# zju3dv/LoFTR

Hardware: AMD Instinct MI355X
Metric: image-pairs/sec @640x480 indoor-ds (higher is better)
Workload: dtype f32; 1 GPU; batch=8 640x480 synthetic grayscale pairs per GPU, indoor_ds dual-softmax (BASELINE configs[1]), full LoFTR.forward = ResNet-FPN backbone (HIP implicit-GEMM / patch convolutions incl. the 7x7 stem) + HIP matching path; weights=seeded random init (no checkpoint on the box), conf_matrix_materialised=True, match_type=dual_softmax, global_batch=8, parallelism=dp1 (pairs sharded; RCCL all-gather of match counts)

## Files before the change

loftr_amd/csrc/common.h:

```cpp
#pragma once
#include <hip/hip_runtime.h>
#include <stdint.h>
#include <stddef.h>
#include "../../include/loftr_hip.h"

typedef float f32x16 __attribute__((ext_vector_type(16)));
typedef float f32x4 __attribute__((ext_vector_type(4)));
typedef float f32x2 __attribute__((ext_vector_type(2)));

#define LOFTR_NEG_INF (-1e9f)

#define LOFTR_CHECK_ARG(cond) do { if (!(cond)) return LOFTR_ERR_BAD_ARG; } while (0)
#define LOFTR_CHECK_LAUNCH() do { if (hipGetLastError() != hipSuccess) return LOFTR_ERR_LAUNCH; } while (0)

#ifdef __HIP_DEVICE_COMPILE__
#define LOFTR_NO_PACKED_FP32 __attribute__((target("no-packed-fp32-ops")))
#else
#define LOFTR_NO_PACKED_FP32
#endif

__host__ __device__ static inline int ceil_div(int a, int b) { return (a + b - 1) / b; }
static inline size_t align_up(size_t x, size_t a) { return (x + a - 1) / a * a; }

enum LoftrTimedKernel {
  LOFTR_T_SCORE_STATS = 0,
  LOFTR_T_SCORE_CONF = 1,
  LOFTR_T_PROJ = 2,
  LOFTR_T_LINEAR = 3,
  LOFTR_T_LINEAR_LN = 4,
  LOFTR_T_KV = 5,
  LOFTR_T_ATTN_APPLY = 6,
  LOFTR_T_ATTN_SMALL = 7,
  LOFTR_T_GATHER = 8,
  LOFTR_T_OT_STORE = 9,
  LOFTR_T_CONV = 10,
  LOFTR_T_CONV3 = 11,
  LOFTR_T_CONV3W = 12,
  LOFTR_T_ENCODER_X = 13,
  LOFTR_T_FINE_PAIR = 14,
  LOFTR_T_COUNT = 15
};
enum LoftrDebugKey {
  LOFTR_DBG_ENCODER_SCHEDULE = 0,
  LOFTR_DBG_CONV_PERSIST_CAP,
  LOFTR_DBG_WGRAD_CHUNK,
  LOFTR_DBG_REDUCE_TALL,
  LOFTR_DBG_PCT_GRID,
  LOFTR_DBG_PCT_SKIP,
  LOFTR_DBG_PCT_QUOTA,
  LOFTR_DBG_CONV_DUO,
  LOFTR_DBG_CONV_PATCH,
  LOFTR_DBG_CONV_REM,
  LOFTR_DBG_FINE_WAVES,
  LOFTR_DBG_COUNT
};
int loftr_debug_value(int key);
extern unsigned g_loftr_timing_mask;
extern int g_loftr_range_check;
void loftr_timing_mark(int id, hipStream_t st, bool end);
struct TimedLaunch {
  int id; hipStream_t st; bool on;
  TimedLaunch(int id_, hipStream_t st_) : id(id_), st(st_), on((g_loftr_timing_mask >> id_) & 1u) {
    if (on) loftr_timing_mark(id, st, false);
  }
  ~TimedLaunch() { if (on) loftr_timing_mark(id, st, true); }
};

constexpr int NUM_XCD = 8;
static inline unsigned xcd_grid(int tiles_m, int tiles_n) { return (unsigned)(NUM_XCD * ceil_div(tiles_m, NUM_XCD) * tiles_n); }
__device__ __forceinline__ bool xcd_tile(int tiles_m, int tiles_n, int& tile_m, int& tile_n) {
  const int id = blockIdx.x, xcd = id % NUM_XCD, slot = id / NUM_XCD;
  const int chunk = ceil_div(tiles_m, NUM_XCD);
  tile_n = slot % tiles_n;
  const int local = slot / tiles_n;
  tile_m = xcd * chunk + local;
  return local < chunk && tile_m < tiles_m;
}

struct WsAlloc {
  char* base; size_t cap; size_t off;
  WsAlloc(void* p, size_t bytes) : base((char*)p), cap(bytes), off(0) {}
  template <typename T> T* take(size_t n) {
    off = align_up(off, 256);
    T* r = (T*)(base + off);
    off += n * sizeof(T);
    return r;
  }
  bool ok() const { return off <= cap; }
};

__device__ __forceinline__ float wave_sum(float v) {
#pragma unroll
  for (int o = 32; o >= 1; o >>= 1) v += __shfl_xor(v, o, 64);
  return v;
}
__device__ __forceinline__ float wave_max(float v) {
#pragma unroll
  for (int o = 32; o >= 1; o >>= 1) v = fmaxf(v, __shfl_xor(v, o, 64));
  return v;
}
#define LOFTR_DPP(v_, ctrl_) __int_as_float(__builtin_amdgcn_update_dpp(0, __float_as_int(v_), ctrl_, 0xF, 0xF, true))
#define LOFTR_DPPI(v_, ctrl_) __builtin_amdgcn_update_dpp(0, v_, ctrl_, 0xF, 0xF, true)
__device__ __forceinline__ float half_sum(float v) {
  v += LOFTR_DPP(v, 0xB1);
  v += LOFTR_DPP(v, 0x4E);
  v += LOFTR_DPP(v, 0x141);
  v += LOFTR_DPP(v, 0x140);
  const auto r = __builtin_amdgcn_permlane16_swap(__float_as_int(v), __float_as_int(v), false, false);
  return __int_as_float(r[0]) + __int_as_float(r[1]);
}
__device__ __forceinline__ float half_max(float v) {
  v = fmaxf(v, LOFTR_DPP(v, 0xB1));
  v = fmaxf(v, LOFTR_DPP(v, 0x4E));
  v = fmaxf(v, LOFTR_DPP(v, 0x141));
  v = fmaxf(v, LOFTR_DPP(v, 0x140));
  const auto r = __builtin_amdgcn_permlane16_swap(__float_as_int(v), __float_as_int(v), false, false);
  return fmaxf(__int_as_float(r[0]), __int_as_float(r[1]));
}
__device__ __forceinline__ int half_min_i32(int v) {
  v = min(v, LOFTR_DPPI(v, 0xB1));
  v = min(v, LOFTR_DPPI(v, 0x4E));
  v = min(v, LOFTR_DPPI(v, 0x141));
  v = min(v, LOFTR_DPPI(v, 0x140));
  const auto r = __builtin_amdgcn_permlane16_swap(v, v, false, false);
  return min((int)r[0], (int)r[1]);
}
__device__ __forceinline__ void half_sum16(f32x16& v) {
#pragma unroll
  for (int r = 0; r < 16; ++r) v[r] += LOFTR_DPP(v[r], 0xB1);
#pragma unroll
  for (int r = 0; r < 16; ++r) v[r] += LOFTR_DPP(v[r], 0x4E);
#pragma unroll
  for (int r = 0; r < 16; ++r) v[r] += LOFTR_DPP(v[r], 0x141);
#pragma unroll
  for (int r = 0; r < 16; ++r) v[r] += LOFTR_DPP(v[r], 0x140);
#pragma unroll
  for (int r = 0; r < 16; ++r) {
    const auto q = __builtin_amdgcn_permlane16_swap(__float_as_int(v[r]), __float_as_int(v[r]), false, false);
    v[r] = __int_as_float(q[0]) + __int_as_float(q[1]);
// ... 27 lines not shown
```

loftr_amd/csrc/conv.hip:

```cpp
#include "gemm.h"
#include "conv_prepared.h"
#include <stdlib.h>

namespace {

using CfgD = GemmCfg<256, 128, 4, 2, 3>;

struct ConvArgs {
  ASrc a;
  const sp_t* w; int K;
  const float* bias;
  const float* wscale;
  const float* x_inv;
  const sp_t* residual;
  sp_t* y_sp;
  float* y_f32;
  int M, Cout, Coutp;
  int act;
  const sp_t* up;
  int Hl, Wl;
  float sy, sx;
};

template <typename Cfg, bool FULL>
__device__ __forceinline__ void conv_epilogue(const ConvArgs& p, f32x16 (&acc)[Cfg::TM][Cfg::TN], int m0, int n0) {
  const EpiLane<Cfg> e;
  const sp_t* rs = p.residual ? p.residual + (long)m0 * p.Coutp + n0 : nullptr;
  sp_t* os = p.y_sp ? p.y_sp + (long)m0 * p.Coutp + n0 : nullptr;
  float* of = p.y_f32 ? p.y_f32 + (long)m0 * p.Cout + n0 : nullptr;
#pragma unroll
  for (int j = 0; j < Cfg::TN; ++j) {
    const int col = n0 + e.lcol + j * 32;
    const bool creal = col < p.Cout;
    const bool cpad = col < p.Coutp;
    const float b = (p.bias && creal) ? p.bias[col] : 0.f;
    const float wsc = (creal ? p.wscale[col] : 1.f) * (p.x_inv ? *p.x_inv : 1.f);
#pragma unroll
    for (int i = 0; i < Cfg::TM; ++i) {
      f32x16 v = acc[i][j] * wsc;
      if (rs) {
        uint32_t w[16];
#pragma unroll
        for (int r = 0; r < 16; ++r) {
          const int trow = e.lrow + e.rr(i, r);
          const bool ok = (FULL || m0 + trow < p.M) && cpad;
          w[r] = ok ? rs[(unsigned)(trow * p.Coutp + e.spcol + j * 32)] : 0u;
        }
#pragma unroll
        for (int r = 0; r < 16; ++r) v[r] += sp_value(w[r], e.odd);
      }
#pragma unroll
      for (int r = 0; r < 16; ++r) {
        float x = v[r] + b;
        if (p.act == 1) x = fmaxf(x, 0.f);
        if (p.act == 2) x = x > 0.f ? x : 0.01f * x;
        v[r] = creal ? x : 0.f;
      }
      if (of) {
#pragma unroll
        for (int r = 0; r < 16; ++r) {
          const int trow = e.lrow + e.rr(i, r);
          if ((FULL || m0 + trow < p.M) && creal) of[(unsigned)(trow * p.Cout + e.lcol + j * 32)] = v[r];
        }
      }
      if (os) {
        uint32_t w[16];
        sp_words16(v, e.odd, w);
#pragma unroll
        for (int r = 0; r < 16; ++r) {
          const int trow = e.lrow + e.rr(i, r);
          if ((FULL || m0 + trow < p.M) && cpad) os[(unsigned)(trow * p.Coutp + e.spcol + j * 32)] = w[r];
        }
      }
    }
  }
}

template <typename Cfg>
__device__ __forceinline__ void conv_epilogue_up(const ConvArgs& p, f32x16 (&acc)[Cfg::TM][Cfg::TN], int m0, int n0,
                                                 float* lds) {
  constexpr int LD = Cfg::BN + 4;
  static_assert(Cfg::BM * LD <= Cfg::LDS_FLOATS, "accumulator tile does not fit the operand ring");
  const EpiLane<Cfg> e;
  __syncthreads();
  const float xinv = p.x_inv ? *p.x_inv : 1.f;
#pragma unroll
  for (int j = 0; j < Cfg::TN; ++j) {
    const int col = n0 + e.lcol + j * 32;
    const float wsc = (col < p.Cout ? p.wscale[col] : 1.f) * xinv;
#pragma unroll
    for (int i = 0; i < Cfg::TM; ++i)
#pragma unroll
      for (int r = 0; r < 16; ++r) lds[(e.lrow + e.rr(i, r)) * LD + e.lcol + j * 32] = acc[i][j][r] * wsc;
  }
  __syncthreads();
  const int Wo = 2 * p.Wl, Ho = 2 * p.Hl;
  constexpr int OCTS = Cfg::BN / 8;
  for (int it = threadIdx.x; it < Cfg::BM * OCTS; it += Cfg::THREADS) {
    const int row = it / OCTS, oct = it - row * OCTS;
    const int pix = m0 + row, col0 = n0 + oct * 8;
    if (pix >= p.M || col0 >= p.Coutp) continue;
    const int t = pix / Wo, x = pix - t * Wo;
    const int bb = t / Ho, y = t - bb * Ho;
    const float fy = p.sy * (float)y, fx = p.sx * (float)x;
    const int y0 = (int)fy, x0 = (int)fx;
    const int dy = y0 < p.Hl - 1 ? p.Wl * p.Coutp : 0, dx = x0 < p.Wl - 1 ? p.Coutp : 0;
    const float ly = fy - (float)y0, lx = fx - (float)x0;
    const float hy = 1.f - ly, hx = 1.f - lx;
    const int off = sp_octet_off(col0 >> 3);
    const sp_t* s00 = p.up + (unsigned)(((bb * p.Hl + y0) * p.Wl + x0) * p.Coutp + off);
    const sp_t* src[4] = {s00, s00 + dx, s00 + dy, s00 + dy + dx};
    u32x4 hi[4], lo[4];
#pragma unroll
    for (int k = 0; k < 4; ++k) {
      hi[k] = *reinterpret_cast<const u32x4*>(src[k]);
      lo[k] = *reinterpret_cast<const u32x4*>(src[k] + 16);
    }
    float v[4][8], o[8];
#pragma unroll
    for (int k = 0; k < 4; ++k) sp_unpack8(hi[k], lo[k], v[k]);
    const f32x4 a0 = *reinterpret_cast<const f32x4*>(&lds[row * LD + oct * 8]);
    const f32x4 a1 = *reinterpret_cast<const f32x4*>(&lds[row * LD + oct * 8 + 4]);
#pragma unroll
    for (int c = 0; c < 8; ++c)
      o[c] = col0 + c < p.Cout
                 ? (c < 4 ? a0[c] : a1[c - 4]) + (hy * (hx * v[0][c] + lx * v[1][c]) + ly * (hx * v[2][c] + lx * v[3][c]))
                 : 0.f;
    u32x4 oh, ol;
    sp_pack8(o, oh, ol);
    sp_t* dst = p.y_sp + (unsigned)(pix * p.Coutp + off);
    *reinterpret_cast<u32x4*>(dst) = oh;
    *reinterpret_cast<u32x4*>(dst + 16) = ol;
  }
}

template <typename Cfg, bool UP>
__global__ __launch_bounds__(Cfg::THREADS, 2) void conv_kernel(ConvArgs p) {
  __shared__ __attribute__((aligned(16))) float lds[Cfg::LDS_FLOATS];
  int tm, tn;
  if (!xcd_tile(ceil_div(p.M, Cfg::BM), ceil_div(p.Coutp, Cfg::BN), tm, tn)) return;
  const int m0 = tm * Cfg::BM, n0 = tn * Cfg::BN;
  f32x16 acc[Cfg::TM][Cfg::TN];
  gemm_mainloop<Cfg, true>(p.a, p.w, p.K, p.M, p.Cout, p.K, m0, n0, lds, acc, p.Coutp);
  if constexpr (UP) conv_epilogue_up<Cfg>(p, acc, m0, n0, lds);
  else if (m0 + Cfg::BM <= p.M) conv_epilogue<Cfg, true>(p, acc, m0, n0);
  else conv_epilogue<Cfg, false>(p, acc, m0, n0);
}

namespace c3 {
constexpr int TY = 8, TX = 32, PW = TX + 2, PH = TY + 2, PROWS = PW * PH;
constexpr int PSLOTS = 43, PQ = 6;
constexpr int PATCH_BYTES = PSLOTS * 1024, BTILE_BYTES = 128 * 128;
constexpr int NB = 4;
constexpr int LDS_BYTES = 2 * PATCH_BYTES + NB * BTILE_BYTES + 1024;
using Cfg = GemmCfg<256, 128, 4, 2, 3>;
}

struct Conv3Args {
  const sp_t* x; int B, H, W, Cp, Cin;
  const sp_t* w; int K;
  const float* bias; const float* wscale; const float* x_inv; const sp_t* residual; sp_t* y_sp; float* y_f32;
  int Cout, Coutp, act;
  const sp_t* zeros;
  int tiles_x, tiles_y;
  float* pbuf;
};

__global__ __launch_bounds__(512, 2) void conv3x3_kernel(Conv3Args p) {
  using namespace c3;
  typedef __attribute__((address_space(3))) void* lds_ptr_t;
  typedef const __attribute__((address_space(1))) void* gbl_ptr_t;
  __shared__ __attribute__((aligned(16))) char lds[LDS_BYTES];
  char* const patch_base = lds;
  char* const bring_base = lds + 2 * PATCH_BYTES;
  char* const scratch = lds + 2 * PATCH_BYTES + NB * BTILE_BYTES;

  const int tid = threadIdx.x, lane = tid & 63, wave = tid >> 6;
  const int wm = wave & 3, wn = wave >> 2;
  const int rsub = lane >> 3, slot = lane & 7;

  const int tiles_m = p.B * p.tiles_y * p.tiles_x, tiles_n = ceil_div(p.Coutp, 128);
  const int chunk_m = ceil_div(tiles_m, NUM_XCD), nvirt = NUM_XCD * chunk_m * tiles_n;
  int vid = blockIdx.x;
  int nb = 0, ny0 = 0, nx0 = 0, nn0 = 0;
  bool have = false;
#define C3_NEXT_TILE()                                                                                      \
  {                                                                                                         \
    have = false;                                                                                           \
    for (; vid < nvirt; vid += gridDim.x) {                                                                 \
      const int xcd__ = vid % NUM_XCD, slot__ = vid / NUM_XCD;                                              \
      const int local__ = slot__ / tiles_n, tm__ = xcd__ * chunk_m + local__;                               \
      if (local__ < chunk_m && tm__ < tiles_m) {                                                            \
        nb = tm__ / (p.tiles_y * p.tiles_x);                                                                \
        const int trem__ = tm__ - nb * (p.tiles_y * p.tiles_x);                                             \
        ny0 = (trem__ / p.tiles_x) * TY; nx0 = (trem__ % p.tiles_x) * TX; nn0 = (slot__ % tiles_n) * 128;   \
        have = true;                                                                                        \
        break;                                                                                              \
      }                                                                                                     \
    }                                                                                                       \
  }
  C3_NEXT_TILE()
  if (!have) return;

  int poff[PQ];
  int boff[2];
#define C3_DMA_OFFSETS()                                                                                    \
  {                                                                                                         \
    _Pragma("unroll") for (int q = 0; q < PQ; ++q) {                                                        \
      const int s = q * 8 + wave, r = s * 8 + rsub;                                                         \
      const int py = r / PW, px = r - py * PW;                                                              \
      const int gy = ny0 - 1 + py, gx = nx0 - 1 + px;                                                       \
      const bool in = s < PSLOTS && r < PROWS && (unsigned)gy < (unsigned)p.H && (unsigned)gx < (unsigned)p.W; \
      poff[q] = in ? ((nb * p.H + gy) * p.W + gx) * p.Cp + ((slot ^ ((r >> 1) & 7)) << 2) : -1;             \
    }                                                                                                       \
    _Pragma("unroll") for (int q = 0; q < 2; ++q) {                                                         \
      const int r = (q * 8 + wave) * 8 + rsub;                                                              \
      boff[q] = min(nn0 + r, p.Cout - 1) * p.K + ((slot ^ ((r >> 1) & 7)) << 2);                            \
    }                                                                                                       \
  }
  C3_DMA_OFFSETS()
  const int gpt = p.Cp >> 5, nk = 9 * gpt;

#define C3_ISSUE_PATCH(cg_, stage_)                                                                         \
  {                                                                                                         \
    _Pragma("unroll") for (int q = 0; q < PQ; ++q) {                                                        \
      const sp_t* g__ = poff[q] >= 0 ? p.x + (poff[q] + (cg_) * 32) : p.zeros;                              \
      char* d__ = (q * 8 + wave < PSLOTS) ? patch_base + (stage_) * PATCH_BYTES + (q * 8 + wave) * 1024 : scratch; \
      __builtin_amdgcn_global_load_lds((gbl_ptr_t)g__, (lds_ptr_t)d__, 16, 0, 0);                           \
    }                                                                                                       \
// ... 384 lines not shown
    cus = per_dev[dev];
  }
  return cus > 0 && nvirt > (unsigned)cus ? (unsigned)cus : nvirt;
}

template <int RT>
__global__ __launch_bounds__(256) void conv_rem_gather_kernel(const float* __restrict__ pbuf, long npix, int H, int W, int R, int c0, int Coutp,
                                                              const float* __restrict__ bias, const sp_t* __restrict__ residual, int act,
                                                              sp_t* __restrict__ y_sp) {
  const long pix = (long)blockIdx.x * 256 + threadIdx.x;
  if (pix >= npix) return;
  const int x = (int)(pix % W), y = (int)((pix / W) % H);
  float v[8];
#pragma unroll
  for (int c = 0; c < 8; ++c) v[c] = 0.f;
  const float* pp = pbuf + pix * (9 * R);
#pragma unroll
  for (int ky = 0; ky < 3; ++ky)
#pragma unroll
    for (int kx = 0; kx < 3; ++kx) {
      const int yy = y + ky - 1, xx = x + kx - 1;
      if ((unsigned)yy < (unsigned)H && (unsigned)xx < (unsigned)W) {
        const float* q = pp + ((long)(ky - 1) * W + (kx - 1)) * (9 * R) + (ky * 3 + kx) * R;
        if (RT == 4) {
          const f32x4 t = *reinterpret_cast<const f32x4*>(q);
          v[0] += t[0]; v[1] += t[1]; v[2] += t[2]; v[3] += t[3];
        } else {
#pragma unroll
          for (int c = 0; c < 7; ++c) if (c < R) v[c] += q[c];
        }
      }
    }
  sp_t* row = y_sp + pix * Coutp + c0;
  float rv[8];
#pragma unroll
  for (int c = 0; c < 8; ++c) rv[c] = 0.f;
  if (residual) {
    const sp_t* rr = residual + pix * Coutp + c0;
    const u32x4 hi = *reinterpret_cast<const u32x4*>(rr), lo = *reinterpret_cast<const u32x4*>(rr + 16);
    sp_unpack8(hi, lo, rv);
  }
  const float slope = act == 1 ? 0.f : act == 2 ? 0.01f : 1.f;
  float o[8];
#pragma unroll
  for (int c = 0; c < 8; ++c) {
    const float t = v[c] + ((bias && c < R) ? bias[c0 + c] : 0.f) + rv[c];
    o[c] = c < R ? fmaxf(t, slope * t) : 0.f;
  }
  u32x4 oh, ol;
  sp_pack8(o, oh, ol);
  const u32x4 z = {0u, 0u, 0u, 0u};
  u32x4* dst = reinterpret_cast<u32x4*>(row);
  dst[0] = oh; dst[1] = z; dst[2] = z; dst[3] = z; dst[4] = ol; dst[5] = z; dst[6] = z; dst[7] = z;
}


static int conv_prepare(const float* weight, const long* weight_strides, int Cin, int Cout, int KH, int KW,
                        const float* bn_weight, const float* bn_bias, const float* bn_mean, const float* bn_var, float bn_eps,
                        void* buf, size_t bytes, hipStream_t st) {
  LOFTR_CHECK_ARG(weight && weight_strides && buf && Cin > 0 && Cout > 0 && KH > 0 && KW > 0);
  LOFTR_CHECK_ARG((bn_weight == nullptr) == (bn_bias == nullptr) && (bn_weight == nullptr) == (bn_mean == nullptr) &&
                  (bn_weight == nullptr) == (bn_var == nullptr));
  ConvPrepared pr;
  if (!conv_prepared_layout(buf, bytes, Cin, Cout, KH, KW, pr)) return LOFTR_ERR_WORKSPACE;
  const int Cp = ceil32(Cin), K = KH * KW * Cp;
  (void)hipMemsetAsync(pr.zeros, 0, 256, st);
  hipLaunchKernelGGL(conv_rowscale_kernel, dim3(Cout), dim3(256), 0, st, weight, bn_weight, bn_bias, bn_mean, bn_var, bn_eps,
                     Cin, KH, KW, weight_strides[0], weight_strides[1], weight_strides[2], weight_strides[3], pr.bias, pr.wscale);
  hipLaunchKernelGGL(conv_prep_kernel, dim3(ceil_div(K / 32, 8), Cout), dim3(256), 0, st, weight, bn_weight, bn_bias,
                     bn_mean, bn_var, bn_eps, Cin, Cp, KH, KW, weight_strides[0], weight_strides[1], weight_strides[2],
                     weight_strides[3], pr.wsp, pr.wscale);
  LOFTR_CHECK_LAUNCH();
  return LOFTR_OK;
}

static int conv_rem_channels(int Cout, int KH, int KW, int stride) {
  return (KH == 3 && KW == 3 && stride == 1 && ceil32(Cout) == 224 && Cout - 192 >= 1 && Cout - 192 <= 7) ? Cout - 192 : 0;
}
extern "C" size_t loftr_conv_scratch_bytes(int B, int H, int W, int Cout, int KH, int KW, int stride) {
  const int R = conv_rem_channels(Cout, KH, KW, stride);
  return (R > 0 && B > 0 && H > 0 && W > 0) ? (size_t)B * H * W * 9 * R * 4 : 0;
}

static int conv_run(const uint32_t* x_sp, int B, int H, int W, int Cin, const void* prepared, size_t prepared_bytes, int Cout,
                    int KH, int KW, int stride, int pad, int act, const uint32_t* residual_sp, const uint32_t* up_sp,
                    uint32_t* y_sp, float* y_f32, void* stream, const float* x_inv = nullptr, void* scratch = nullptr, size_t scratch_bytes = 0) {
  LOFTR_CHECK_ARG(x_sp && prepared && (y_sp || y_f32) && B >= 0 && H > 0 && W > 0 && Cin > 0 && Cout > 0);
  const bool shared_gpu = (act & LOFTR_CONV_SHARED_GPU) != 0;
  act &= ~LOFTR_CONV_SHARED_GPU;
  LOFTR_CHECK_ARG(KH > 0 && KW > 0 && stride > 0 && pad >= 0 && act >= 0 && act <= 2);
  if (B == 0) return LOFTR_OK;
  hipStream_t st = (hipStream_t)stream;
  ConvGeom g;
  g.H = H; g.W = W; g.Cp = ceil32(Cin); g.KH = KH; g.KW = KW; g.stride = stride; g.pad = pad;
  g.Ho = (H + 2 * pad - KH) / stride + 1;
  g.Wo = (W + 2 * pad - KW) / stride + 1;
  if (g.Ho <= 0 || g.Wo <= 0 || H >= 32768 || W >= 32768) return LOFTR_ERR_UNSUPPORTED;
  if (up_sp && ((g.Ho & 1) || (g.Wo & 1) || KH != 1 || KW != 1 || stride != 1 || pad != 0 || !y_sp || y_f32 || residual_sp || act != 0))
    return LOFTR_ERR_UNSUPPORTED;
  const long M = (long)B * g.Ho * g.Wo;
  if (M * (long)ceil32(Cout) >= (1L << 31) || (long)B * H * W * g.Cp >= (1L << 31)) return LOFTR_ERR_UNSUPPORTED;
  const int K = KH * KW * g.Cp;
  ConvPrepared pr;
  if (!conv_prepared_layout(const_cast<void*>(prepared), prepared_bytes, Cin, Cout, KH, KW, pr)) return LOFTR_ERR_WORKSPACE;
  sp_t* wsp = pr.wsp;
  float* bias = pr.bias;
  sp_t* zeros = pr.zeros;
  g.zeros = zeros;
  ConvArgs p;
  p.a = asrc_conv(x_sp, g);
  p.w = wsp; p.K = K; p.bias = bias; p.wscale = pr.wscale; p.x_inv = x_inv; p.residual = residual_sp; p.y_sp = y_sp; p.y_f32 = y_f32;
  p.M = (int)M; p.Cout = Cout; p.Coutp = ceil32(Cout); p.act = act;
  p.up = up_sp; p.Hl = g.Ho / 2; p.Wl = g.Wo / 2;
  p.sy = g.Ho > 1 ? (float)(p.Hl - 1) / (float)(g.Ho - 1) : 0.f;
  p.sx = g.Wo > 1 ? (float)(p.Wl - 1) / (float)(g.Wo - 1) : 0.f;
  if (loftr_debug_value(LOFTR_DBG_CONV_PATCH) && KH == 3 && KW == 3 && stride == 1 && pad == 1 && !up_sp) {
    Conv3Args c;
    c.x = x_sp; c.B = B; c.H = H; c.W = W; c.Cp = g.Cp; c.Cin = Cin; c.w = wsp; c.K = K; c.bias = bias; c.wscale = pr.wscale; c.x_inv = x_inv; c.residual = residual_sp;
    c.y_sp = y_sp; c.y_f32 = y_f32; c.Cout = Cout; c.Coutp = ceil32(Cout); c.act = act; c.zeros = zeros;
    c.tiles_x = ceil_div(W, c3::TX); c.tiles_y = ceil_div(H, c3::TY); c.pbuf = nullptr;
    const bool duo = loftr_debug_value(LOFTR_DBG_CONV_DUO) != 0;
    const bool wide = duo && c.Coutp == 32 * 7;
    TimedLaunch tl(wide ? LOFTR_T_CONV3W : LOFTR_T_CONV3, st);
    if (duo && c.Coutp % 128 == 0) {
      using CF = c3d::Cfg<4, 2, 4>;
      c.tiles_y = ceil_div(H, CF::TY);
      hipLaunchKernelGGL((conv3x3_duo_kernel<CF>), dim3(xcd_grid(B * c.tiles_x * c.tiles_y, c.Coutp / 128)), dim3(256), 0, st, c);
    } else if (duo && c.Coutp == 192) {
      using CF = c3d::Cfg<6, 2, 4, 8, 2>;
      c.tiles_y = ceil_div(H, CF::TY);
      hipLaunchKernelGGL((conv3x3_duo_kernel<CF>), dim3(xcd_grid(B * c.tiles_x * c.tiles_y, 1)), dim3(512), 0, st, c);
    } else if (wide && conv_rem_channels(Cout, KH, KW, stride) > 0 && !y_f32 && loftr_debug_value(LOFTR_DBG_CONV_REM) &&
               scratch && scratch_bytes >= (size_t)B * H * W * 9 * conv_rem_channels(Cout, KH, KW, stride) * 4) {
      using CF = c3d::Cfg<6, 2, 4, 8, 2, true>;
      c.tiles_y = ceil_div(H, CF::TY);
      c.pbuf = reinterpret_cast<float*>(scratch);
      hipLaunchKernelGGL((conv3x3_duo_kernel<CF>), dim3(xcd_grid(B * c.tiles_x * c.tiles_y, 1)), dim3(512), 0, st, c);
      LOFTR_CHECK_LAUNCH();
      const long npix = (long)B * H * W;
      if (Cout - 192 == 4)
        hipLaunchKernelGGL(conv_rem_gather_kernel<4>, dim3((unsigned)((npix + 255) / 256)), dim3(256), 0, st, c.pbuf, npix, H, W, 4, 192, c.Coutp,
                           bias, residual_sp, act, y_sp);
      else
        hipLaunchKernelGGL(conv_rem_gather_kernel<0>, dim3((unsigned)((npix + 255) / 256)), dim3(256), 0, st, c.pbuf, npix, H, W, Cout - 192, 192, c.Coutp,
                           bias, residual_sp, act, y_sp);
    } else if (wide) {
      using CF = c3d::Cfg<7, 2, 4, 8, 2>;
      c.tiles_y = ceil_div(H, CF::TY);
      hipLaunchKernelGGL((conv3x3_duo_kernel<CF>), dim3(xcd_grid(B * c.tiles_x * c.tiles_y, 1)), dim3(512), 0, st, c);
    } else
      hipLaunchKernelGGL(conv3x3_kernel, dim3(shared_gpu ? xcd_grid(B * c.tiles_x * c.tiles_y, ceil_div(c.Coutp, 128))
                                                         : persistent_grid(xcd_grid(B * c.tiles_x * c.tiles_y, ceil_div(c.Coutp, 128)))),
                         dim3(512), 0, st, c);
    LOFTR_CHECK_LAUNCH();
    return LOFTR_OK;
  }
  {
    TimedLaunch tl(LOFTR_T_CONV, st);
    if (up_sp)
      hipLaunchKernelGGL((conv_kernel<CfgD, true>), dim3(xcd_grid(ceil_div(p.M, CfgD::BM), ceil_div(p.Coutp, CfgD::BN))),
                         dim3(CfgD::THREADS), 0, st, p);
    else
      hipLaunchKernelGGL((conv_kernel<CfgD, false>), dim3(xcd_grid(ceil_div(p.M, CfgD::BM), ceil_div(p.Coutp, CfgD::BN))),
                         dim3(CfgD::THREADS), 0, st, p);
  }
  LOFTR_CHECK_LAUNCH();
  return LOFTR_OK;
}

#ifdef LOFTR_CONV_PROBE
extern "C" int loftr_conv_probe_buffer(void* buf) {
  long long* b = (long long*)buf;
  return hipMemcpyToSymbol(HIP_SYMBOL(g_conv_probe), &b, sizeof(b)) == hipSuccess ? LOFTR_OK : LOFTR_ERR_LAUNCH;
}
#endif

extern "C" int loftr_conv_prepare(const float* weight, const long* weight_strides, int Cin, int Cout, int KH, int KW,
                                  const float* bn_weight, const float* bn_bias, const float* bn_mean, const float* bn_var,
                                  float bn_eps, void* prepared, size_t prepared_bytes, void* stream) {
  return conv_prepare(weight, weight_strides, Cin, Cout, KH, KW, bn_weight, bn_bias, bn_mean, bn_var, bn_eps, prepared,
                      prepared_bytes, (hipStream_t)stream);
}

extern "C" int loftr_conv_bn_act_prepared(const uint32_t* x_sp, int B, int H, int W, int Cin, const void* prepared,
                                          size_t prepared_bytes, int Cout, int KH, int KW, int stride, int pad, int act,
                                          const uint32_t* residual_sp, const uint32_t* low_sp, uint32_t* y_sp, float* y_f32,
                                          const float* x_inv_scale, void* stream) {
  return conv_run(x_sp, B, H, W, Cin, prepared, prepared_bytes, Cout, KH, KW, stride, pad, act, residual_sp, low_sp, y_sp, y_f32,
                  stream, x_inv_scale);
}

extern "C" int loftr_conv_bn_act_prepared_scratch(const uint32_t* x_sp, int B, int H, int W, int Cin, const void* prepared,
                                                  size_t prepared_bytes, int Cout, int KH, int KW, int stride, int pad, int act,
                                                  const uint32_t* residual_sp, const uint32_t* low_sp, uint32_t* y_sp, float* y_f32,
                                                  const float* x_inv_scale, void* scratch, size_t scratch_bytes, void* stream) {
  return conv_run(x_sp, B, H, W, Cin, prepared, prepared_bytes, Cout, KH, KW, stride, pad, act, residual_sp, low_sp, y_sp, y_f32,
                  stream, x_inv_scale, scratch, scratch_bytes);
}

extern "C" int loftr_conv_bn_act(const uint32_t* x_sp, int B, int H, int W, int Cin, const float* weight,
                                 const long* weight_strides, int Cout, int KH, int KW, int stride, int pad, const float* bn_weight, const float* bn_bias,
                                 const float* bn_mean, const float* bn_var, float bn_eps, int act,
                                 const uint32_t* residual_sp, uint32_t* y_sp, float* y_f32, void* ws, size_t ws_bytes,
                                 const float* x_inv_scale, void* stream) {
  LOFTR_CHECK_ARG(x_sp && (y_sp || y_f32) && B >= 0 && H > 0 && W > 0);
  if (B == 0) return LOFTR_OK;
  const int rc = conv_prepare(weight, weight_strides, Cin, Cout, KH, KW, bn_weight, bn_bias, bn_mean, bn_var, bn_eps, ws, ws_bytes,
                              (hipStream_t)stream);
  if (rc != LOFTR_OK) return rc;
  return conv_run(x_sp, B, H, W, Cin, ws, ws_bytes, Cout, KH, KW, stride, pad, act, residual_sp, nullptr, y_sp, y_f32, stream, x_inv_scale);
}

extern "C" int loftr_conv1x1_upsample_add(const uint32_t* x_sp, int B, int H, int W, int Cin, const float* weight,
                                          const long* weight_strides, int Cout, const uint32_t* low_sp, uint32_t* y_sp,
                                          void* ws, size_t ws_bytes, void* stream) {
  LOFTR_CHECK_ARG(x_sp && low_sp && y_sp && B >= 0 && H > 0 && W > 0);
  if (B == 0) return LOFTR_OK;
  const int rc = conv_prepare(weight, weight_strides, Cin, Cout, 1, 1, nullptr, nullptr, nullptr, nullptr, 0.f, ws, ws_bytes,
                              (hipStream_t)stream);
  if (rc != LOFTR_OK) return rc;
  return conv_run(x_sp, B, H, W, Cin, ws, ws_bytes, Cout, 1, 1, 1, 0, 0, nullptr, low_sp, y_sp, nullptr, stream);
}

extern "C" int loftr_stem_conv_bn_relu(const float* x, const long* x_strides, int B, int H, int W, const float* weight,
                                       const long* weight_strides, int C0, const float* bn_weight, const float* bn_bias,
                                       const float* bn_mean, const float* bn_var, float bn_eps, uint32_t* y_sp,
                                       void* stream) {
  LOFTR_CHECK_ARG(x && x_strides && weight && weight_strides && y_sp && B >= 0 && H > 0 && W > 0 && C0 > 0);
  LOFTR_CHECK_ARG((bn_weight == nullptr) == (bn_bias == nullptr) && (bn_weight == nullptr) == (bn_mean == nullptr) &&
                  (bn_weight == nullptr) == (bn_var == nullptr));
  if (C0 > 128) return LOFTR_ERR_UNSUPPORTED;
  if (B == 0) return LOFTR_OK;
  const int Ho = (H + 6 - 7) / 2 + 1, Wo = (W + 6 - 7) / 2 + 1;
  hipLaunchKernelGGL(stem_conv_kernel, dim3(ceil_div(Wo, STEM_TX), ceil_div(Ho, STEM_TY), B), dim3(256), 0,
                     (hipStream_t)stream, x, x_strides[0], x_strides[2], x_strides[3], H, W, weight, weight_strides[0],
                     weight_strides[2], weight_strides[3], bn_weight, bn_bias, bn_mean, bn_var, bn_eps, C0, Ho, Wo, y_sp);
  LOFTR_CHECK_LAUNCH();
  return LOFTR_OK;
}
// ... 36 lines not shown
```

loftr_amd/csrc/misc.hip:

```cpp
#include "common.h"
#include <string.h>

namespace {
template <bool CL>
__global__ void pos_encode_flatten_kernel(loftr_fmap f, const float* __restrict__ pe,
                                          int pe_h, int pe_w, float* __restrict__ out, int C) {
  __shared__ float tile[32][33];
  const int H = f.H, W = f.W, HW = H * W;
  const int n = blockIdx.z, hw0 = blockIdx.x * 32, c0 = blockIdx.y * 32;
  const float* in = f.data + (long)n * f.sn;
  for (int k = threadIdx.y; k < 32; k += 8) {
    const int c = c0 + k, hw = hw0 + threadIdx.x;
    float v = 0.f;
    if (c < C && hw < HW) {
      const int y = hw / W, x = hw - y * W;
      v = pe[((long)c * pe_h + y) * pe_w + x];
      if (!CL) v += in[(long)c * f.sc + (long)y * f.sh + (long)x * f.sw];
    }
    tile[k][threadIdx.x] = v;
  }
  __syncthreads();
  for (int k = threadIdx.y; k < 32; k += 8) {
    const int hw = hw0 + k, c = c0 + threadIdx.x;
    if (hw < HW && c < C) {
      float v = tile[threadIdx.x][k];
      if (CL) { const int y = hw / W, x = hw - y * W; v += in[(long)y * f.sh + (long)x * f.sw + c]; }
      out[((long)n * HW + hw) * C + c] = v;
    }
  }
}
}

extern "C" int loftr_pos_encode_flatten(const loftr_fmap* feat, const float* pe, int pe_h, int pe_w, float* out,
                                        int N, int C, void* stream) {
  LOFTR_CHECK_ARG(feat && feat->data && pe && out && N >= 0 && C > 0 && feat->H > 0 && feat->W > 0 &&
                  feat->H <= pe_h && feat->W <= pe_w);
  if (N == 0) return LOFTR_OK;
  const dim3 grid(ceil_div(feat->H * feat->W, 32), ceil_div(C, 32), N), block(32, 8);
  if (feat->sc == 1)
    hipLaunchKernelGGL((pos_encode_flatten_kernel<true>), grid, block, 0, (hipStream_t)stream, *feat, pe, pe_h, pe_w, out, C);
  else
    hipLaunchKernelGGL((pos_encode_flatten_kernel<false>), grid, block, 0, (hipStream_t)stream, *feat, pe, pe_h, pe_w, out, C);
  LOFTR_CHECK_LAUNCH();
  return LOFTR_OK;
}

namespace {
struct DebugSwitch { const char* name; int def; int value; };
DebugSwitch g_debug[LOFTR_DBG_COUNT] = {{"encoder_schedule", 1, 1}, {"conv_persist_cap", 0, 0}, {"wgrad_chunk", 0, 0}, {"reduce_tall", 1, 1},
                                        {"pct_grid", 0, 0}, {"pct_skip", 0, 0}, {"pct_quota", 0, 0}, {"conv_duo", 1, 1}, {"conv_patch", 1, 1}, {"conv_rem", 1, 1},
                                        {"fine_waves", 0, 0}};
}
int loftr_debug_value(int key) { return (key >= 0 && key < LOFTR_DBG_COUNT) ? g_debug[key].value : 0; }
extern "C" int loftr_hip_debug_set(const char* key, int value) {
  LOFTR_CHECK_ARG(key != nullptr);
  for (auto& d : g_debug)
    if (strcmp(d.name, key) == 0) { d.value = value; return LOFTR_OK; }
  return LOFTR_ERR_BAD_ARG;
}
extern "C" int loftr_hip_debug_get(const char* key, int* value, int* default_value) {
  LOFTR_CHECK_ARG(key != nullptr && value != nullptr);
  for (auto& d : g_debug)
    if (strcmp(d.name, key) == 0) { *value = d.value; if (default_value) *default_value = d.def; return LOFTR_OK; }
  return LOFTR_ERR_BAD_ARG;
}

unsigned g_loftr_timing_mask = 0;
int g_loftr_range_check = 0;
extern "C" int loftr_hip_range_check_enable(int on) { g_loftr_range_check = on ? 1 : 0; return LOFTR_OK; }
namespace {
constexpr int T_POOL = 4096;
struct TimingSlot {
  hipEvent_t ev[T_POOL][2];
  int created, used;
  double total_ms; long long launches;
};
TimingSlot g_slots[LOFTR_T_COUNT];
const char* const T_NAMES[LOFTR_T_COUNT] = {"score_sweep_kernel<0>", "score_sweep_kernel<1>", "proj_kernel", "linear_kernel",
                                            "linear_ln_kernel", "proj_kv_kernel", "attn_apply_kernel",
                                            "attn_small_kernel", "gather_windows_kernel", "score_sweep_kernel<2>", "conv_kernel",
                                            "conv3x3_duo_kernel<Cfg<4,2,4,4,1>>", "conv3x3_duo_kernel<Cfg<7,2,4,8,2>>", "encoder_x_kernel", "fine_pair_kernel"};
void timing_drain(TimingSlot& s) {
  for (int i = 0; i < s.used; ++i) {
    float ms = 0.f;
    if (hipEventSynchronize(s.ev[i][1]) == hipSuccess && hipEventElapsedTime(&ms, s.ev[i][0], s.ev[i][1]) == hipSuccess) {
      s.total_ms += ms;
      s.launches += 1;
    }
  }
  s.used = 0;
}
}

void loftr_timing_mark(int id, hipStream_t st, bool end) {
  TimingSlot& s = g_slots[id];
  if (!end) {
    if (s.used >= T_POOL) return;
    if (s.used >= s.created) {
      if (hipEventCreate(&s.ev[s.created][0]) != hipSuccess || hipEventCreate(&s.ev[s.created][1]) != hipSuccess) return;
      s.created++;
    }
    (void)hipEventRecord(s.ev[s.used][0], st);
  } else {
    if (s.used >= s.created) return;
    (void)hipEventRecord(s.ev[s.used][1], st);
    s.used++;
  }
}

extern "C" int loftr_hip_timing_enable(unsigned mask) {
  g_loftr_timing_mask = mask & ((1u << LOFTR_T_COUNT) - 1u);
  return LOFTR_OK;
}

extern "C" int loftr_hip_timing_kernel_count(void) { return LOFTR_T_COUNT; }

extern "C" const char* loftr_hip_timing_kernel_name(int id) {
  return (id >= 0 && id < LOFTR_T_COUNT) ? T_NAMES[id] : "";
}

extern "C" int loftr_hip_timing_read(int id, double* total_ms, long long* launches, int reset) {
  LOFTR_CHECK_ARG(id >= 0 && id < LOFTR_T_COUNT && total_ms && launches);
  TimingSlot& s = g_slots[id];
  timing_drain(s);
  *total_ms = s.total_ms;
  *launches = s.launches;
  if (reset) { s.total_ms = 0.0; s.launches = 0; }
  return LOFTR_OK;
}

extern "C" int loftr_hip_abi_version(void) { return LOFTR_HIP_ABI_VERSION; }

extern "C" const char* loftr_hip_status_string(int status) {
  switch (status) {
    case LOFTR_OK: return "ok";
    case LOFTR_ERR_BAD_ARG: return "bad argument (null pointer or invalid shape)";
// ... 18 lines not shown
```

Measured before the change: 470.2 image-pairs/s.

## Add full-width 256x256 conv tile kernel for 224/256-channel convolutions

Adds a conv kernel whose tile covers the whole output-channel width (BM=256, BN=256) for layers with 224 or 256 padded output channels. It uses split-fp16 MFMA with separate A/B LDS rings and an optional deeper A prefetch. The upsample epilogue is reworked to park 64-column slices in the dead LDS ring. The path is picked by a CU-count wave-quantisation heuristic comparing full-width tiles to two half-width tiles, and is on by default. The aim is to load each A tile once instead of twice and to reduce tail-wave waste, at the cost of fewer blocks, higher register and LDS use, and lower occupancy.

```diff
diff --git a/loftr_amd/csrc/common.h b/loftr_amd/csrc/common.h
--- a/loftr_amd/csrc/common.h
+++ b/loftr_amd/csrc/common.h
@@ -52,9 +52,12 @@
   LOFTR_DBG_CONV_PATCH,
   LOFTR_DBG_CONV_REM,
   LOFTR_DBG_FINE_WAVES,
+  LOFTR_DBG_CONV_FULL,
+  LOFTR_DBG_CONV_LAST,
   LOFTR_DBG_COUNT
 };
 int loftr_debug_value(int key);
+void loftr_debug_record(int key, int value);
 extern unsigned g_loftr_timing_mask;
 extern int g_loftr_range_check;
 void loftr_timing_mark(int id, hipStream_t st, bool end);
diff --git a/loftr_amd/csrc/conv.hip b/loftr_amd/csrc/conv.hip
--- a/loftr_amd/csrc/conv.hip
+++ b/loftr_amd/csrc/conv.hip
@@ -1,5 +1,6 @@
 #include "gemm.h"
 #include "conv_prepared.h"
+#include "conv_full_map.h"
 #include <stdlib.h>
 
 namespace {
@@ -22,7 +23,7 @@
   float sy, sx;
 };
 
-template <typename Cfg, bool FULL>
+template <typename Cfg, bool FULL, bool TRIM = false>
 __device__ __forceinline__ void conv_epilogue(const ConvArgs& p, f32x16 (&acc)[Cfg::TM][Cfg::TN], int m0, int n0) {
   const EpiLane<Cfg> e;
   const sp_t* rs = p.residual ? p.residual + (long)m0 * p.Coutp + n0 : nullptr;
@@ -30,6 +31,9 @@
   float* of = p.y_f32 ? p.y_f32 + (long)m0 * p.Cout + n0 : nullptr;
 #pragma unroll
   for (int j = 0; j < Cfg::TN; ++j) {
+    if constexpr (TRIM) {
+      if (n0 + (int)(threadIdx.x >> 6) / Cfg::WM * Cfg::WTN + j * 32 >= p.Coutp) continue;
+    }
     const int col = n0 + e.lcol + j * 32;
     const bool creal = col < p.Cout;
     const bool cpad = col < p.Coutp;
@@ -76,6 +80,38 @@
   }
 }
 
+__device__ __forceinline__ void conv_up_item(const ConvArgs& p, int pix, int col0, const f32x4& a0, const f32x4& a1, int Wo, int Ho) {
+  const int t = pix / Wo, x = pix - t * Wo;
+  const int bb = t / Ho, y = t - bb * Ho;
+  const float fy = p.sy * (float)y, fx = p.sx * (float)x;
+  const int y0 = (int)fy, x0 = (int)fx;
+  const int dy = y0 < p.Hl - 1 ? p.Wl * p.Coutp : 0, dx = x0 < p.Wl - 1 ? p.Coutp : 0;
+  const float ly = fy - (float)y0, lx = fx - (float)x0;
+  const float hy = 1.f - ly, hx = 1.f - lx;
+  const int off = sp_octet_off(col0 >> 3);
+  const sp_t* s00 = p.up + (unsigned)(((bb * p.Hl + y0) * p.Wl + x0) * p.Coutp + off);
+  const sp_t* src[4] = {s00, s00 + dx, s00 + dy, s00 + dy + dx};
+  u32x4 hi[4], lo[4];
+#pragma unroll
+  for (int k = 0; k < 4; ++k) {
+    hi[k] = *reinterpret_cast<const u32x4*>(src[k]);
+    lo[k] = *reinterpret_cast<const u32x4*>(src[k] + 16);
+  }
+  float v[4][8], o[8];
+#pragma unroll
+  for (int k = 0; k < 4; ++k) sp_unpack8(hi[k], lo[k], v[k]);
+#pragma unroll
+  for (int c = 0; c < 8; ++c)
+    o[c] = col0 + c < p.Cout
+               ? (c < 4 ? a0[c] : a1[c - 4]) + (hy * (hx * v[0][c] + lx * v[1][c]) + ly * (hx * v[2][c] + lx * v[3][c]))
+               : 0.f;
+  u32x4 oh, ol;
+  sp_pack8(o, oh, ol);
+  sp_t* dst = p.y_sp + (unsigned)(pix * p.Coutp + off);
+  *reinterpret_cast<u32x4*>(dst) = oh;
+  *reinterpret_cast<u32x4*>(dst + 16) = ol;
+}
+
 template <typename Cfg>
 __device__ __forceinline__ void conv_epilogue_up(const ConvArgs& p, f32x16 (&acc)[Cfg::TM][Cfg::TN], int m0, int n0,
                                                  float* lds) {
@@ -100,37 +136,9 @@
     const int row = it / OCTS, oct = it - row * OCTS;
     const int pix = m0 + row, col0 = n0 + oct * 8;
     if (pix >= p.M || col0 >= p.Coutp) continue;
-    const int t = pix / Wo, x = pix - t * Wo;
-    const int bb = t / Ho, y = t - bb * Ho;
-    const float fy = p.sy * (float)y, fx = p.sx * (float)x;
-    const int y0 = (int)fy, x0 = (int)fx;
-    const int dy = y0 < p.Hl - 1 ? p.Wl * p.Coutp : 0, dx = x0 < p.Wl - 1 ? p.Coutp : 0;
-    const float ly = fy - (float)y0, lx = fx - (float)x0;
-    const float hy = 1.f - ly, hx = 1.f - lx;
-    const int off = sp_octet_off(col0 >> 3);
-    const sp_t* s00 = p.up + (unsigned)(((bb * p.Hl + y0) * p.Wl + x0) * p.Coutp + off);
-    const sp_t* src[4] = {s00, s00 + dx, s00 + dy, s00 + dy + dx};
-    u32x4 hi[4], lo[4];
-#pragma unroll
-    for (int k = 0; k < 4; ++k) {
-      hi[k] = *reinterpret_cast<const u32x4*>(src[k]);
-      lo[k] = *reinterpret_cast<const u32x4*>(src[k] + 16);
-    }
-    float v[4][8], o[8];
-#pragma unroll
-    for (int k = 0; k < 4; ++k) sp_unpack8(hi[k], lo[k], v[k]);
     const f32x4 a0 = *reinterpret_cast<const f32x4*>(&lds[row * LD + oct * 8]);
     const f32x4 a1 = *reinterpret_cast<const f32x4*>(&lds[row * LD + oct * 8 + 4]);
-#pragma unroll
-    for (int c = 0; c < 8; ++c)
-      o[c] = col0 + c < p.Cout
-                 ? (c < 4 ? a0[c] : a1[c - 4]) + (hy * (hx * v[0][c] + lx * v[1][c]) + ly * (hx * v[2][c] + lx * v[3][c]))
-                 : 0.f;
-    u32x4 oh, ol;
-    sp_pack8(o, oh, ol);
-    sp_t* dst = p.y_sp + (unsigned)(pix * p.Coutp + off);
-    *reinterpret_cast<u32x4*>(dst) = oh;
-    *reinterpret_cast<u32x4*>(dst + 16) = ol;
+    conv_up_item(p, pix, col0, a0, a1, Wo, Ho);
   }
 }
 
@@ -145,6 +153,156 @@
   if constexpr (UP) conv_epilogue_up<Cfg>(p, acc, m0, n0, lds);
   else if (m0 + Cfg::BM <= p.M) conv_epilogue<Cfg, true>(p, acc, m0, n0);
   else conv_epilogue<Cfg, false>(p, acc, m0, n0);
+}
+
+using CfgF = GemmCfg<256, 256, 4, 2, 2>;
+static_assert(CfgF::WTM == cfmap::WTM && CfgF::WTN == cfmap::WTN && CfgF::TM == cfmap::TM && CfgF::TN == cfmap::TN && CfgF::WM == cfmap::WM &&
+              CfgF::A_DMA == cfmap::QA && CfgF::B_DMA == cfmap::QB && CfgF::TILE_A == cfmap::TILE_BYTES, "conv_full_map.h restates this tile");
+
+template <int NJ>
+__device__ __forceinline__ void conv_full_compute(const char* sA, const char* sB, int a_r0, int b_r0, int g, f32x16 (&acc)[2][4]) {
+#pragma unroll
+  for (int ks = 0; ks < 2; ++ks) {
+    h16x8 ah[2], al[2], bh[NJ], bl[NJ];
+#pragma unroll
+    for (int i = 0; i < 2; ++i) {
+      ah[i] = *reinterpret_cast<const h16x8*>(sA + cfmap::frag_off(a_r0 + i * 32, ks * 2 + g));
+      al[i] = *reinterpret_cast<const h16x8*>(sA + cfmap::frag_off(a_r0 + i * 32, 4 + ks * 2 + g));
+    }
+#pragma unroll
+    for (int j = 0; j < NJ; ++j) {
+      bh[j] = *reinterpret_cast<const h16x8*>(sB + cfmap::frag_off(b_r0 + j * 32, ks * 2 + g));
+      bl[j] = *reinterpret_cast<const h16x8*>(sB + cfmap::frag_off(b_r0 + j * 32, 4 + ks * 2 + g));
+    }
+#pragma unroll
+    for (int i = 0; i < 2; ++i)
+#pragma unroll
+      for (int j = 0; j < NJ; ++j) acc[i][j] = __builtin_amdgcn_mfma_f32_32x32x16_f16(al[i], bh[j], acc[i][j], 0, 0, 0);
+#pragma unroll
+    for (int i = 0; i < 2; ++i)
+#pragma unroll
+      for (int j = 0; j < NJ; ++j) acc[i][j] = __builtin_amdgcn_mfma_f32_32x32x16_f16(ah[i], bl[j], acc[i][j], 0, 0, 0);
+#pragma unroll
+    for (int i = 0; i < 2; ++i)
+#pragma unroll
+      for (int j = 0; j < NJ; ++j) acc[i][j] = __builtin_amdgcn_mfma_f32_32x32x16_f16(ah[i], bh[j], acc[i][j], 0, 0, 0);
+  }
+}
+
+template <int NSA, int NSB>
+__device__ __forceinline__ void conv_full_mainloop(const ConvArgs& p, int m0, char* lds, f32x16 (&acc)[2][4]) {
+  using namespace cfmap;
+  static_assert(NSB >= 2 && (NSA == NSB || NSA == NSB + 1), "A is issued NSA - 1 k-tiles ahead, B NSB - 1");
+  typedef __attribute__((address_space(3))) void* lds_ptr_t;
+  typedef const __attribute__((address_space(1))) void* gbl_ptr_t;
+  char* ldsB = lds + NSA * TILE_BYTES;
+  const int lane = threadIdx.x & 63, wave = threadIdx.x >> 6;
+  const ConvGeom& cv = p.a.cv;
+  int aoff[QA], ayx[QA], boff[QB];
+#pragma unroll
+  for (int q = 0; q < QA; ++q) {
+    const int r = dma_row(q, wave, lane);
+    const APix px = a_pixel(cv, min(m0 + r, p.M - 1), dma_chunk(r, lane));
+    aoff[q] = px.off; ayx[q] = px.ayx;
+  }
+#pragma unroll
+  for (int q = 0; q < QB; ++q) {
+    const int r = dma_row(q, wave, lane);
+    boff[q] = b_off(r, p.Cout, p.K, dma_chunk(r, lane));
+  }
+  KPos kp{0, 0, 0, 0};
+#define CF_ISSUE_A(stage_)                                                                                  \
+  {                                                                                                         \
+    char* s__ = lds + (stage_) * TILE_BYTES + wave * 1024;                                                  \
+    _Pragma("unroll") for (int q = 0; q < QA; ++q) {                                                        \
+      const sp_t* g__ = a_inside(cv, ayx[q], kp) ? p.a.p0 + (aoff[q] + kp.toff) : cv.zeros;                 \
+      __builtin_amdgcn_global_load_lds((gbl_ptr_t)g__, (lds_ptr_t)(s__ + q * WAVES * 1024), 16, 0, 0);      \
+    }                                                                                                       \
+    k_advance(cv, kp);                                                                                      \
+  }
+#define CF_ISSUE_B(kt_, stage_)                                                                             \
+  {                                                                                                         \
+    char* s__ = ldsB + (stage_) * TILE_BYTES + wave * 1024;                                                 \
+    _Pragma("unroll") for (int q = 0; q < QB; ++q)                                                          \
+      if (b_live(q, wave, p.Coutp))                                                       \
+        __builtin_amdgcn_global_load_lds((gbl_ptr_t)(p.w + (boff[q] + (kt_) * 32)), (lds_ptr_t)(s__ + q * WAVES * 1024), 16, 0, 0); \
+  }
+#pragma unroll
+  for (int i = 0; i < 2; ++i)
+#pragma unroll
+    for (int j = 0; j < 4; ++j)
+#pragma unroll
+      for (int r = 0; r < 16; ++r) acc[i][j][r] = 0.f;
+
+  const int g = lane >> 5;
+  const int a_r0 = wave_m(wave) * WTM + (lane & 31);
+  const int b_r0 = wave_n(wave) * WTN + (lane & 31);
+  const int nj = live_tiles(wave_n(wave), p.Coutp);
+  const int nk = p.K / 32;
+  CF_ISSUE_A(0);
+  CF_ISSUE_B(0, 0);
+  if (NSA > NSB && nk > 1) CF_ISSUE_A(1);
+  int sa = 0, sb = 0, ia = NSA - 1, ib = NSB - 1;
+  for (int kt = 0; kt < nk; ++kt) {
+    if (NSA > NSB && kt + 1 < nk) LOFTR_WAITCNT_VM(QA);
+    else LOFTR_WAITCNT_VM(0);
+    __builtin_amdgcn_s_barrier();
+    if (kt + NSB - 1 < nk) CF_ISSUE_B(kt + NSB - 1, ib);
+    if (kt + NSA - 1 < nk) CF_ISSUE_A(ia);
+    const char* sA = lds + sa * TILE_BYTES;
+    const char* sB = ldsB + sb * TILE_BYTES;
+    if (nj == 4) conv_full_compute<4>(sA, sB, a_r0, b_r0, g, acc);
+    else conv_full_compute<3>(sA, sB, a_r0, b_r0, g, acc);
+    sa = sa + 1 == NSA ? 0 : sa + 1;
+    sb = sb + 1 == NSB ? 0 : sb + 1;
+    ia = ia + 1 == NSA ? 0 : ia + 1;
+    ib = ib + 1 == NSB ? 0 : ib + 1;
+  }
+  __builtin_amdgcn_s_barrier();
+#undef CF_ISSUE_A
+#undef CF_ISSUE_B
+}
+
+__device__ __forceinline__ void conv_full_epilogue_up(const ConvArgs& p, f32x16 (&acc)[2][4], int m0, float* lds) {
+  using namespace cfmap;
+  const int lane = threadIdx.x & 63, wave = threadIdx.x >> 6;
+  const float xinv = p.x_inv ? *p.x_inv : 1.f;
+  const int Wo = 2 * p.Wl, Ho = 2 * p.Hl;
+#pragma unroll
+  for (int s = 0; s < SLICES; ++s) {
+    __syncthreads();
+    if (wave_n(wave) * WTN + s * 32 < p.Coutp) {
+      const int col = acc_col(wave, lane, s);
+      const float wsc = (col < p.Cout ? p.wscale[col] : 1.f) * xinv;
+#pragma unroll
+      for (int i = 0; i < 2; ++i)
+#pragma unroll
+        for (int r = 0; r < 16; ++r) lds[acc_row(wave, lane, i, r) * SLICE_LD + slice_park_col(wave, lane)] = acc[i][s][r] * wsc;
+    }
+    __syncthreads();
+    for (int it = threadIdx.x; it < BM * SLICE_OCTS; it += 512) {
+      const int row = it / SLICE_OCTS, oct = it - row * SLICE_OCTS;
+      const int pix = m0 + row, col0 = slice_col0(s, oct);
+      if (pix >= p.M || col0 >= p.Coutp) continue;
+      const f32x4 a0 = *reinterpret_cast<const f32x4*>(&lds[row * SLICE_LD + oct * 8]);
+      const f32x4 a1 = *reinterpret_cast<const f32x4*>(&lds[row * SLICE_LD + oct * 8 + 4]);
+      conv_up_item(p, pix, col0, a0, a1, Wo, Ho);
+    }
+  }
+}
+
+template <int NSA, int NSB, bool UP>
+__global__ __launch_bounds__(512) void conv_full_kernel(ConvArgs p) {
+  static_assert(cfmap::BM * cfmap::SLICE_LD * 4 <= (NSA + NSB) * cfmap::TILE_BYTES, "a parked slice must fit the dead ring");
+  __shared__ __attribute__((aligned(16))) float lds[(NSA + NSB) * cfmap::TILE_BYTES / 4];
+  int tm, tn;
+  if (!xcd_tile(ceil_div(p.M, cfmap::BM), 1, tm, tn)) return;
+  const int m0 = tm * cfmap::BM;
+  f32x16 acc[2][4];
+  conv_full_mainloop<NSA, NSB>(p, m0, reinterpret_cast<char*>(lds), acc);
+  if constexpr (UP) conv_full_epilogue_up(p, acc, m0, lds);
+  else if (m0 + cfmap::BM <= p.M) conv_epilogue<CfgF, true, true>(p, acc, m0, 0);
+  else conv_epilogue<CfgF, false, true>(p, acc, m0, 0);
 }
 
 namespace c3 {
@@ -695,6 +853,26 @@
   return (R > 0 && B > 0 && H > 0 && W > 0) ? (size_t)B * H * W * 9 * R * 4 : 0;
 }
 
+static int device_cus() {
+  static int per_dev[64];
+  int dev = 0, n = 0;
+  if (hipGetDevice(&dev) != hipSuccess || dev < 0 || dev >= 64) return 0;
+  if (per_dev[dev] == 0) {
+    if (hipDeviceGetAttribute(&n, hipDeviceAttributeMultiprocessorCount, dev) != hipSuccess) return 0;
+    per_dev[dev] = n;
+  }
+  return per_dev[dev];
+}
+static int conv_full_ring(long M, int Coutp) {
+  const int sw = loftr_debug_value(LOFTR_DBG_CONV_FULL);
+  if (sw <= 0 || (Coutp != 224 && Coutp != 256)) return 0;
+  if (sw >= 2) return sw == 2 ? 1 : 2;
+  const long cus = device_cus(), T = (M + cfmap::BM - 1) / cfmap::BM;
+  if (cus <= 0) return 0;
+  const long full = (T + cus - 1) / cus * (Coutp / 32), halves = (2 * T + cus - 1) / cus * 4;
+  return full <= halves ? 2 : 0;
+}
+
 static int conv_run(const uint32_t* x_sp, int B, int H, int W, int Cin, const void* prepared, size_t prepared_bytes, int Cout,
                     int KH, int KW, int stride, int pad, int act, const uint32_t* residual_sp, const uint32_t* up_sp,
                     uint32_t* y_sp, float* y_f32, void* stream, const float* x_inv = nullptr, void* scratch = nullptr, size_t scratch_bytes = 0) {
@@ -728,6 +906,7 @@
   p.sy = g.Ho > 1 ? (float)(p.Hl - 1) / (float)(g.Ho - 1) : 0.f;
   p.sx = g.Wo > 1 ? (float)(p.Wl - 1) / (float)(g.Wo - 1) : 0.f;
   if (loftr_debug_value(LOFTR_DBG_CONV_PATCH) && KH == 3 && KW == 3 && stride == 1 && pad == 1 && !up_sp) {
+    loftr_debug_record(LOFTR_DBG_CONV_LAST, -1);
     Conv3Args c;
     c.x = x_sp; c.B = B; c.H = H; c.W = W; c.Cp = g.Cp; c.Cin = Cin; c.w = wsp; c.K = K; c.bias = bias; c.wscale = pr.wscale; c.x_inv = x_inv; c.residual = residual_sp;
     c.y_sp = y_sp; c.y_f32 = y_f32; c.Cout = Cout; c.Coutp = ceil32(Cout); c.act = act; c.zeros = zeros;
@@ -768,6 +947,21 @@
     LOFTR_CHECK_LAUNCH();
     return LOFTR_OK;
   }
+  const int full = conv_full_ring(M, p.Coutp);
+  loftr_debug_record(LOFTR_DBG_CONV_LAST, full);
+  if (full) {
+    TimedLaunch tl(LOFTR_T_CONV, st);
+    const dim3 grid(xcd_grid(ceil_div(p.M, cfmap::BM), 1)), block(512);
+    if (full == 1) {
+      if (up_sp) hipLaunchKernelGGL((conv_full_kernel<3, 2, true>), grid, block, 0, st, p);
+      else hipLaunchKernelGGL((conv_full_kernel<3, 2, false>), grid, block, 0, st, p);
+    } else {
+      if (up_sp) hipLaunchKernelGGL((conv_full_kernel<2, 2, true>), grid, block, 0, st, p);
+      else hipLaunchKernelGGL((conv_full_kernel<2, 2, false>), grid, block, 0, st, p);
+    }
+    LOFTR_CHECK_LAUNCH();
+    return LOFTR_OK;
+  }
   {
     TimedLaunch tl(LOFTR_T_CONV, st);
     if (up_sp)
diff --git a/loftr_amd/csrc/conv_full_map.h b/loftr_amd/csrc/conv_full_map.h
--- /dev/null
+++ b/loftr_amd/csrc/conv_full_map.h
@@ -0,0 +1,52 @@
+#pragma once
+#if defined(__HIPCC__)
+#define CF_HD __host__ __device__ __forceinline__
+#else
+#define CF_HD static inline
+#endif
+
+namespace cfmap {
+constexpr int BM = 256, BN = 256, WAVES = 8, WM = 4, WTM = 64, WTN = 128, TM = 2, TN = 4;
+constexpr int QA = 4, QB = 4;
+constexpr int TILE_BYTES = 256 * 128;
+constexpr int SLICES = 4, SLICE_COLS = 64, SLICE_LD = SLICE_COLS + 4, SLICE_OCTS = SLICE_COLS / 8;
+
+CF_HD int dma_row(int q, int wave, int lane) { return (q * WAVES + wave) * 8 + (lane >> 3); }
+CF_HD int dma_chunk(int r, int lane) { return (lane & 7) ^ ((r >> 1) & 7); }
+CF_HD int dma_lds_off(int q, int wave, int lane) { return (q * WAVES + wave) * 1024 + lane * 16; }
+CF_HD int frag_off(int r, int c) { return r * 128 + ((c ^ ((r >> 1) & 7)) << 4); }
+
+struct APix { int off, ayx; };
+template <class G> CF_HD APix a_pixel(const G& g, int gr, int chunk) {
+  const int hw = g.Ho * g.Wo;
+  const int b = gr / hw, rem = gr - b * hw;
+  const int yo = rem / g.Wo, xo = rem - yo * g.Wo;
+  const int yb = yo * g.stride - g.pad, xb = xo * g.stride - g.pad;
+  return APix{((b * g.H + yb) * g.W + xb) * g.Cp + chunk * 4, (int)(((unsigned)yb << 16) | ((unsigned)xb & 0xffffu))};
+}
+struct KPos { int cg, ky, kx, toff; };
+template <class G> CF_HD void k_advance(const G& g, KPos& k) {
+  k.toff += 32;
+  if (++k.cg == g.Cp / 32) {
+    k.cg = 0;
+    if (++k.kx == g.KW) { k.kx = 0; ++k.ky; k.toff += (g.W - g.KW) * g.Cp; }
+  }
+}
+template <class G> CF_HD bool a_inside(const G& g, int ayx, const KPos& k) {
+  const int y = (ayx >> 16) + k.ky, x = (int)(short)(ayx & 0xffff) + k.kx;
+  return (unsigned)y < (unsigned)g.H && (unsigned)x < (unsigned)g.W;
+}
+
+CF_HD bool b_live(int q, int wave, int Coutp) { return (q * WAVES + wave) * 8 < Coutp; }
+CF_HD int b_off(int r, int Cout, int K, int chunk) { return (r < Cout ? r : Cout - 1) * K + chunk * 4; }
+
+CF_HD int wave_m(int wave) { return wave % WM; }
+CF_HD int wave_n(int wave) { return wave / WM; }
+CF_HD int live_tiles(int wn, int Coutp) { const int n = (Coutp - wn * WTN) / 32; return n < TN ? n : TN; }
+CF_HD int acc_row(int wave, int lane, int i, int reg) { return wave_m(wave) * WTM + 4 * (lane >> 5) + i * 32 + (reg & 3) + 8 * (reg >> 2); }
+CF_HD int acc_col(int wave, int lane, int j) { return wave_n(wave) * WTN + j * 32 + (lane & 31); }
+CF_HD int acc_spcol(int wave, int lane, int j) { return wave_n(wave) * WTN + j * 32 + ((lane & 1) ? 16 : 0) + ((lane & 31) >> 1); }
+
+CF_HD int slice_park_col(int wave, int lane) { return wave_n(wave) * 32 + (lane & 31); }
+CF_HD int slice_col0(int s, int oct) { return (oct >> 2) * WTN + s * 32 + (oct & 3) * 8; }
+}
diff --git a/loftr_amd/csrc/misc.hip b/loftr_amd/csrc/misc.hip
--- a/loftr_amd/csrc/misc.hip
+++ b/loftr_amd/csrc/misc.hip
@@ -49,9 +49,10 @@
 struct DebugSwitch { const char* name; int def; int value; };
 DebugSwitch g_debug[LOFTR_DBG_COUNT] = {{"encoder_schedule", 1, 1}, {"conv_persist_cap", 0, 0}, {"wgrad_chunk", 0, 0}, {"reduce_tall", 1, 1},
                                         {"pct_grid", 0, 0}, {"pct_skip", 0, 0}, {"pct_quota", 0, 0}, {"conv_duo", 1, 1}, {"conv_patch", 1, 1}, {"conv_rem", 1, 1},
-                                        {"fine_waves", 0, 0}};
+                                        {"fine_waves", 0, 0}, {"conv_full", 1, 1}, {"conv_last", 0, 0}};
 }
 int loftr_debug_value(int key) { return (key >= 0 && key < LOFTR_DBG_COUNT) ? g_debug[key].value : 0; }
+void loftr_debug_record(int key, int value) { if (key >= 0 && key < LOFTR_DBG_COUNT) g_debug[key].value = value; }
 extern "C" int loftr_hip_debug_set(const char* key, int value) {
   LOFTR_CHECK_ARG(key != nullptr);
   for (auto& d : g_debug)
```

Result: no change. 467.2 image-pairs/s (median of 2 runs) (-0.6%).
